# SeoYeonnLee/Video-Chapter-Generation

Hardware: AMD Instinct MI355X
Metric: clip-windows/sec (16f×224²+128tok) train-step at 1/2/4/8 MI355X; % HBM roofline (higher is better)
Workload: dtype bf16; 1 GPU; TwoStream train step: TSM-ResNet-50 + BERT-base + ChapterHead(mlp), B=64 windows/GPU of 16x224^2 frames + 128 tokens, fused clip+AdamW; global_batch=64, seq_len=128, frames=16, resolution=224, text_fill=n_valid ~ U[L/2, L], parallelism=dp1

## Files before the change

include/vcg_hip.h:

```cpp
#ifndef VCG_HIP_H
#define VCG_HIP_H
#include <hip/hip_runtime.h>
#include <stdint.h>
#ifdef __cplusplus
extern "C" {
#endif

#define VCG_API
enum { VCG_F32 = 0, VCG_BF16 = 1 };
enum { VCG_GRAD_F32 = 0x10 };
enum { VCG_OK = 0, VCG_ERR_INVALID = -1, VCG_ERR_UNSUPPORTED = -2, VCG_ERR_HIP = -3 };
enum { VCG_ACT_NONE = 0, VCG_ACT_RELU = 1, VCG_ACT_GELU = 2, VCG_ACT_TANH = 3, VCG_ACT_GELU_BWD = 4 };
enum { VCG_ACT_FLAG_ROUND_PRE = 0x100 };
enum { VCG_ACT_FLAG_WIDE = 0x200 };
enum { VCG_ACT_FLAG_F32_OUT = 0x400 };
VCG_API int vcg_gemm_census_enable(int on);
VCG_API int vcg_gemm_census_size(void);
VCG_API int vcg_gemm_census_get(int i, char* key, int n, long long* count);

VCG_API const char* vcg_last_error(void);
VCG_API int vcg_version(void);
VCG_API int vcg_init(int device);
VCG_API int vcg_finalize(void);
VCG_API int vcg_sync(hipStream_t stream);
VCG_API int vcg_timing_enable(int on);
VCG_API int vcg_timing_query(int kernel_id, double* ms_total, long long* launches, double* flops);
VCG_API int vcg_timing_roofline(int kernel_id, double peak_tflops, double peak_gbs, double* ms_total, double* ideal_ms, double* bytes, double* flops);
VCG_API int vcg_patch_stamps(unsigned long long* out, int n);
VCG_API int vcg_fast_stamps(unsigned long long* out, int n);
VCG_API int vcg_g256_stamps(unsigned long long* out, int n);
VCG_API int vcg_wide_stamps(unsigned long long* out, int n);

VCG_API int vcg_conv_stats_tiles(int M);
VCG_API int vcg_conv_fwd(int dtype, const void* x, const void* w, void* y, float* stats, int N, int H, int W, int C, int Cout, int KH, int KW, int stride, int pad, int tsm_T, int tsm_fold, hipStream_t stream);
VCG_API int vcg_conv_fwd_bias_act(int dtype, const void* x, const void* w, const float* bias, int act, void* y, int N, int H, int W, int C, int Cout, int KH, int KW, int stride, int pad, int tsm_T, int tsm_fold, hipStream_t stream);
VCG_API int vcg_conv_dgrad(int dtype, const void* dy, const void* wt, void* dx, int N, int H, int W, int C, int Cout, int KH, int KW, int stride, int pad, hipStream_t stream);
VCG_API long long vcg_conv_dgrad_bwd_ws_bytes(int C, int Cout, int KH, int KW);
VCG_API long long vcg_conv_dgrad_bwd_p_ws_bytes(int C, int a2_c);
VCG_API int vcg_conv_dgrad_bwd(int dtype, const void* dy, const void* wt, void* g, int N, int H, int W, int C, int Cout, int KH, int KW, int stride, int pad, int tsm_T, int tsm_fold, const void* res, int res_stride, const unsigned char* bits, const void* y, const float* mean, const float* invstd, const float* mscale, const float* mshift, const void* y2, const float* mean2, const float* invstd2, float* ws, long long ws_bytes, float* sum_g, float* sum_gx, float* dgamma, float* dbeta, float* sum_gx2, float* dgamma2, float* dbeta2, const void* a2, int a2_c, float* pg, float* pws, long long pws_bytes, hipStream_t s);
VCG_API long long vcg_conv_wgrad_ws_bytes(int dtype, int N, int H, int W, int C, int Cout, int KH, int KW, int stride, int pad);
VCG_API int vcg_conv_wgrad(int dtype, const void* x, const void* dy, float* dw, int accumulate, float* ws, long long ws_bytes, int N, int H, int W, int C, int Cin, int Cout, int KH, int KW, int stride, int pad, int tsm_T, int tsm_fold, hipStream_t stream);
VCG_API int vcg_conv1x1_bn_res_relu(const void* x, const void* wfold, const float* bias, const void* res, const float* res_scale, const float* res_shift, void* out, unsigned char* bits, int M, int N, int K, hipStream_t stream);
VCG_API int vcg_bn_bwd_fold_weights(const void* wt, int N, int K, const float* mean, const float* invstd, const float* gamma, const float* sum_g, const float* sum_gx, float inv_count, void* wfold, float* bias, hipStream_t stream);
VCG_API long long vcg_bn_apply_colsum_ws_bytes(long long P, int C);
VCG_API int vcg_bn_apply_colsum(const void* y, const float* scale, const float* shift, int relu, void* out, float* colsum, float* ws, long long ws_bytes, long long P, int C, hipStream_t s);
VCG_API long long vcg_bn_apply_gram_ws_bytes(long long P, int C);
VCG_API int vcg_bn_apply_gram(const void* y, const float* scale, const float* shift, const float* mean, const float* invstd, void* out, float* colsum, float* gram, double* g64, float* ws, long long ws_bytes, long long P, int C, hipStream_t s);
VCG_API int vcg_bn_stats_from_gram(const double* g64, const void* w, long long M, int N, int C, float* stats, int mtiles, hipStream_t s);
VCG_API int vcg_bn_finalize_from_gram(const double* g64, const void* w, long long M, int N, int C, const float* gamma,
                                      const float* beta, float* mean, float* invstd, float* scale, float* shift,
                                      float* running_mean, float* running_var, float momentum, float eps,
                                      const float* w32, void* wfold, hipStream_t s);
VCG_API int vcg_conv1x1_stats(const void* x, const void* w, float* stats, int M, int N, int K, hipStream_t stream);
VCG_API int vcg_bn_bwd_sumgx_from_wgrad(const float* P, const void* w, int K, int C, const float* mean, const float* invstd, const float* sum_g, float* sum_gx, float* dgamma, hipStream_t stream);
VCG_API int vcg_bn_bwd_fold_weights_a2(const void* wt, int C, int K, const float* invstd, const float* gamma, const float* sum_g, const float* sum_gx, float inv_count, const float* colsum_a, void* wfold, float* bias, hipStream_t stream);
VCG_API int vcg_bn_bwd_fold_wgrad_a2(const float* P, const float* G, const float* w3, int K, int C, const float* mean, const float* invstd, const float* gamma, const float* sum_g, const float* sum_gx, float inv_count, const float* colsum_a, float* dw, int accumulate, hipStream_t stream);
VCG_API int vcg_conv_dgrad_bwd_bnfold(const void* g, const void* yg, int Ky, const void* wfold, const float* bias, void* out, int N, int H, int W, int C, int Cout, const void* y, const float* mean, const float* invstd, const float* mscale, const float* mshift, float* ws, long long ws_bytes, float* sum_g, float* sum_gx, float* dgamma, float* dbeta, hipStream_t stream);
VCG_API long long vcg_conv_wgrad_bnfold_ws_bytes(int N, int H, int W, int C, int Cout);
// ... 113 lines not shown
```

video-chapter-generation_amd/csrc/igemm.h:

```cpp
#pragma once
#include "common.h"

namespace vcg {

enum { OP_DENSE_K = 0, OP_IM2COL = 1, OP_DGRAD = 2, OP_DENSE_MN = 3, OP_IM2COL_T = 4 };
enum { EPI_STORE = 0, EPI_STATS = 1, EPI_SPLITK = 2, EPI_BWD = 3, EPI_BWD_AFF = 4, EPI_STORE_AUX = 5,
       EPI_BWD_STREAM = 6 };
enum { ACT_NONE = 0, ACT_RELU = 1, ACT_GELU = 2, ACT_TANH = 3, ACT_GELU_BWD = 4 };
enum { ACT_FLAG_ROUND_PRE = 0x100 };
enum { ACT_FLAG_WIDE = 0x200 };
enum { ACT_FLAG_F32_OUT = 0x400 };

template <typename T> struct Cfg;
template <> struct Cfg<float> { static constexpr int VEC = 4, BK = 16, LDK = 20; };
template <> struct Cfg<bf16_t> { static constexpr int VEC = 8, BK = 32, LDK = 40; };

template <typename T, int COLS> struct LdMN {
  static constexpr int v = sizeof(T) == 2 ? (COLS == 128 ? 144 : 80) : (COLS == 128 ? 132 : 68);
};

constexpr bool is_kcontig(int mode) { return mode == OP_DENSE_K || mode == OP_IM2COL || mode == OP_DGRAD; }

struct OpArgs {
  const void* ptr;
// ... 197 lines not shown
            const float mb = red[2 * BN + lc], d = mb - mean, nt = n1 + n2;
            mean += d * (n2 / nt);
            m2 += red[3 * BN + lc] + d * d * (n1 * n2 / nt);
          }
          reinterpret_cast<float2*>(p.stats)[(long long)col * mtiles + mtile] = make_float2(mean, m2);
        }
    }
    if (blockIdx.x == 0 && threadIdx.x == 0)
      reinterpret_cast<float2*>(p.stats)[(long long)p.N * mtiles + mtile] =
          make_float2((float)min(BM, p.M - m0), 0.f);
#pragma unroll
    for (int j = 0; j < NT; ++j) {
      const int n = nbase + j * 16;
#pragma unroll
      for (int i = 0; i < MT; ++i) {
        const int m = mbase + i * 16;
        if (m >= p.M || n >= p.N) continue;
        float v[4] = {acc[i][j][0], acc[i][j][1], acc[i][j][2], acc[i][j][3]};
        store4<T>(Cout + (long long)m * p.ldc + n, v);
      }
    }
  }
}

int run_fast_gemm(GemmParams& p, int amode, int epi, int z, hipStream_t s);
int fast_grid_rows(int M, int N, int z, int epi);
bool fast_bwd_streams(const GemmParams& p);
int wide_gemm_class(const GemmParams& p);
int wide_gemm_class_f32(const GemmParams& p);
int run_gemm_wide(GemmParams& p, int we, hipStream_t s);
int fast_bwd_slots(const GemmParams& p);
int bn_bwd_finalize_launch(const float* partial, int nb, int C, long long ld, int gx_off, float* sum_g, float* sum_gx,
                           float* dgamma, float* dbeta, int accumulate, hipStream_t s);
int run_fast_wgrad(const GemmParams& p, int splits, hipStream_t s, bool dense_b = false);
int wgrad_patch_rows(int dtype, int H, int W, int C, int Cin, int Cout, int KH, int KW, int stride, int pad,
                     int tsm_fold);
int wgrad_patch_splits(int C, int Cout);
int run_rs1x1_bnres(const void* x, const void* wfold, const float* bias, const void* res, void* out, uint8_t* bits,
                    long long M, int N, int K, hipStream_t s);
int run_wgrad_patch(const void* x, const void* dy, float* ws, int N, int H, int W, int C, int Cout, int R,
                    hipStream_t s);
int wgrad_fast_tile_m(int M);
int wgrad_fast_tile_n(int N);

bool gemm256_ok(const GemmParams& p, int amode, int epi, int z);
int run_gemm256(const GemmParams& p, int amode, int epi, hipStream_t s);

}
```

video-chapter-generation_amd/csrc/igemm.hip:

```cpp
#include <cstdio>

#include "igemm.h"

namespace vcg {

template <typename T, int ROWS, int MODE> struct Loader {
  static constexpr int VEC = Cfg<T>::VEC, BK = Cfg<T>::BK;
  static constexpr int NC = ROWS * 4 / 256;
  static constexpr bool KC = is_kcontig(MODE);
  static constexpr int CPR = ROWS / VEC;

  uint4 reg[NC];
  const T* ptr[NC];
  int ra[NC], rb[NC], rc[NC];
  int sub[NC];
  int lds_off[NC];

  __device__ __forceinline__ void init(const OpArgs& a, int row0, int tid) {
    const T* base = reinterpret_cast<const T*>(a.ptr);
#pragma unroll
    for (int j = 0; j < NC; ++j) {
      const int q = tid + j * 256;
      if constexpr (KC) {
        const int row = q >> 2;
// ... 881 lines not shown
  p.K = K;
  p.k_per_split = kps;
  p.a = dense_op(dy, Cout, Cout);
  p.a.bytes = (long long)K * Cout * (dtype == VCG_BF16 ? 2 : 4);
  OpArgs b{};
  b.ptr = x; b.rows = Nn; b.N = N; b.H = H; b.W = W; b.C = C; b.logC = logC;
  b.bytes = (long long)N * H * W * C * (dtype == VCG_BF16 ? 2 : 4);
  b.GH = OH; b.GW = OW; b.KH = KH; b.KW = KW; b.stride = stride; b.pad = pad;
  b.tsm_T = tsm_T > 0 ? tsm_T : 1; b.tsm_fold = tsm_fold;
  b.fd_ghw = make_fastdiv(OH * OW); b.fd_gw = make_fastdiv(OW); b.fd_T = make_fastdiv(b.tsm_T);
  if (pair) {
    b.W = W / 2; b.C = 8; b.logC = 3; b.KW = KWp; b.sw = 1; b.pw = pwp;
  }
  p.b = b;
  p.ws = ws;
  p.alpha = 1.f;
  const int wpr = wgrad_patch_rows(dtype, H, W, C, Cin, Cout, KH, KW, stride, pad, tsm_fold);
  if (wpr > 0) {
    const int wsp = wgrad_patch_splits(C, Cout);
    VCG_REQUIRE(ws_bytes >= (long long)wsp * M * Nn * 4, "workspace too small");
    if (FILE* f = gemm_log())
      fprintf(f, "a=3 b=4 epi=2 M=%d N=%d K=%d z=%d fast=3 conv=%dx%d/%d C=%d\n", M, Nn, K, wsp, KH, KW, stride, C);
    int rc = run_wgrad_patch(x, dy, ws, N, H, W, C, Cout, wpr, stream);
    if (rc) return rc;
    const long long MN = (long long)M * Nn;
    splitk_reduce(stream, ws, wsp, MN,
                       Nn, dw, accumulate, 1, KH, KW, C, Cin, 1.f, KW, 0, pad);
    VCG_LAUNCH_CHECK();
    return VCG_OK;
  }
  FILE* f = fast ? gemm_log() : nullptr;
  if (f)
    fprintf(f, "a=3 b=4 epi=2 M=%d N=%d K=%d z=%d fast=2 conv=%dx%d/%d C=%d\n", M, Nn, K, splits, KH, KW, stride, C);
  int rc;
  if (fast)
    rc = run_fast_wgrad(p, splits, stream);
  else
    rc = dtype == VCG_BF16 ? run_gemm<bf16_t, OP_DENSE_MN, OP_IM2COL_T>(p, EPI_SPLITK, splits, stream)
                           : run_gemm<float, OP_DENSE_MN, OP_IM2COL_T>(p, EPI_SPLITK, splits, stream);
  if (rc) return rc;
  const long long MN = (long long)M * Nn;
  splitk_reduce(stream, ws, splits,
                     MN, Nn, dw, accumulate, pair ? 2 : 1, KH, KW, C, Cin, 1.f, KWp, pwp, pad);
  VCG_LAUNCH_CHECK();
  return VCG_OK;
}

namespace {
__global__ __launch_bounds__(256) void bn_fold_weights_kernel(const bf16_t* __restrict__ wt, int K,
                                                              const float* __restrict__ mean,
                                                              const float* __restrict__ invstd,
                                                              const float* __restrict__ gamma,
                                                              const float* __restrict__ sum_g,
                                                              const float* __restrict__ sum_gx, float ic,
                                                              bf16_t* __restrict__ wf, float* __restrict__ bias) {
  __shared__ float red[256];
  const int n = blockIdx.x, t = threadIdx.x;
  float acc = 0.f;
  for (int k = t; k < K; k += 256) {
    const float is = invstd[k], A = (gamma ? gamma[k] : 1.f) * is;
    const float B = -A * is * sum_gx[k] * ic;
    const float w = bf2f(wt[(long long)n * K + k]);
    const bf16_t wy = f2bf(B * w);
    wf[(long long)n * 2 * K + k] = f2bf(A * w);
    wf[(long long)n * 2 * K + K + k] = wy;
    acc += (-A * sum_g[k] * ic) * w - mean[k] * bf2f(wy);
  }
  red[t] = acc;
  __syncthreads();
  for (int o = 128; o > 0; o >>= 1) {
    if (t < o) red[t] += red[t + o];
    __syncthreads();
  }
  if (t == 0) bias[n] = red[0];
}
// ... 264 lines not shown

VCG_API int vcg_conv_wgrad_bnfold(const void* x, const void* g, const void* yg, const float* mean, const float* invstd,
                                  const float* gamma, const float* sum_g, const float* sum_gx, float inv_count,
                                  const float* colsum_x, float* dw, int accumulate, float* ws, long long ws_bytes, int N,
                                  int H, int W, int C, int Cout, hipStream_t stream) {
  VCG_REQUIRE(x && g && yg && mean && invstd && sum_g && sum_gx && colsum_x && dw, "null argument");
  const int logC = ilog2_exact(C);
  VCG_REQUIRE(logC >= 6 && Cout % 128 == 0, "C must be a power of two >= 64, Cout a multiple of 128");
  int M, Nn, K, splits, kps;
  bool fast;
  wgrad_geometry(VCG_BF16, N, H, W, C, 2 * Cout, 1, 1, 1, 0, &M, &Nn, &K, &splits, &kps, &fast);
  if (!fast || wgrad_fast_tile_m(M) != 128 || (long long)K * Cout * 2 >= 0xFFFFFF00LL) return VCG_ERR_UNSUPPORTED;
  VCG_REQUIRE(ws_bytes >= (long long)splits * M * Nn * 4, "workspace too small");
  GemmParams p{};
  p.M = M;
  p.N = Nn;
  p.K = K;
  p.k_per_split = kps;
  p.a = dense_op(g, Cout, Cout);
  p.a.bytes = (long long)K * Cout * 2;
  p.a.ptr2 = yg;
  p.a.split2 = Cout;
  OpArgs b{};
  b.ptr = x; b.rows = Nn; b.N = N; b.H = H; b.W = W; b.C = C; b.logC = logC;
  b.bytes = (long long)N * H * W * C * 2;
  b.GH = H; b.GW = W; b.KH = 1; b.KW = 1; b.stride = 1; b.pad = 0;
  b.tsm_T = 1; b.tsm_fold = 0;
  b.fd_ghw = make_fastdiv(H * W); b.fd_gw = make_fastdiv(W); b.fd_T = make_fastdiv(1);
  p.b = b;
  p.ws = ws;
  p.alpha = 1.f;
  if (FILE* f = gemm_log())
    fprintf(f, "a=3 b=4 epi=2 M=%d N=%d K=%d z=%d fast=2 conv=1x1/1 C=%d bnfold=1\n", M, Nn, K, splits, C);
  int rc = run_fast_wgrad(p, splits, stream);
  if (rc) return rc;
  const long long MN = (long long)Cout * Nn;
  if ((MN + 255) / 256 < 1024 && splits >= 16)
    hipLaunchKernelGGL(splitk_reduce_bnfold_kernel<8>, dim3((unsigned)((MN * 8 + 255) / 256)), dim3(256), 0, stream,
                       ws, splits, Cout, Nn, mean, invstd, gamma, sum_g, sum_gx, inv_count, colsum_x, dw, accumulate);
  else
    hipLaunchKernelGGL(splitk_reduce_bnfold_kernel<1>, dim3((unsigned)((MN + 255) / 256)), dim3(256), 0, stream, ws,
                       splits, Cout, Nn, mean, invstd, gamma, sum_g, sum_gx, inv_count, colsum_x, dw, accumulate);
  VCG_LAUNCH_CHECK();
  return VCG_OK;
}

VCG_API int vcg_conv1x1_stats(const void* x, const void* w, float* stats, int M, int N, int K, hipStream_t stream) {
  VCG_REQUIRE(x && w && stats, "null argument");
  VCG_REQUIRE(M > 0 && N % 64 == 0 && K % 64 == 0, "N and K must be multiples of 64");
  if (!fast_gemm_enabled() || (long long)M * K * 2 >= 0xFFFFFF00LL) return VCG_ERR_UNSUPPORTED;
  GemmParams p{};
  p.M = M;
  p.N = N;
  p.K = K;
  p.k_per_split = K + 64;
  p.a = dense_op(x, K, M, K, 2);
  p.b = dense_op(w, K, N, K, 2);
  p.C = nullptr;
  p.ldc = N;
  p.alpha = 1.f;
  p.stats = stats;
  if (FILE* f = gemm_log()) {
    fprintf(f, "a=0 b=0 epi=1 M=%d N=%d K=%d z=1 fast=1 conv=1x1/1 C=%d nostore=1\n", M, N, K, K);
    fflush(f);
  }
  const int rc = run_fast_gemm(p, OP_DENSE_K, EPI_STATS, 1, stream);
  return rc < 0 ? VCG_ERR_UNSUPPORTED : rc;
}
// ... 92 lines not shown
  const int splits = choose_splits(M, N, K, dtype == VCG_BF16 ? 32 : 16, VCG_SPLITK_TARGET_DENSE);
  return (long long)splits * M * N * 4;
}

VCG_API int vcg_gemm_splitk(int dtype, int transA, int transB, int M, int N, int K, const void* A, long long lda,
                            const void* B, long long ldb, float* out, int accumulate, float* ws, long long ws_bytes,
                            hipStream_t stream) {
  const int BK = dtype == VCG_BF16 ? 32 : 16;
  int splits = choose_splits(M, N, K, BK, VCG_SPLITK_TARGET_DENSE);
  VCG_REQUIRE(ws_bytes >= (long long)splits * M * N * 4, "workspace too small");
  int kps = (K + splits - 1) / splits;
  kps = (kps + BK - 1) / BK * BK;
  splits = (K + kps - 1) / kps;
  GemmParams p{};
  p.M = M; p.N = N; p.K = K; p.k_per_split = kps;
  p.a = dense_op(A, lda, M);
  p.b = dense_op(B, ldb, N);
  p.ws = ws;
  p.alpha = 1.f;
  int rc;
  const long long a_ext = ((long long)(K - 1) * lda + M) * 2, b_ext = ((long long)(K - 1) * ldb + N) * 2;
  if (dtype == VCG_BF16 && transA && transB && fast_gemm_enabled() &&
      M % 8 == 0 && N % 8 == 0 && lda % 8 == 0 && ldb % 8 == 0 && a_ext < 0xFFFFFF00LL && b_ext < 0xFFFFFF00LL) {
    p.a.bytes = a_ext;
    p.b.bytes = b_ext;
    int fk = (K + splits - 1) / splits;
    fk = (fk + 63) / 64 * 64;
    const int fsplits = (K + fk - 1) / fk;
    p.k_per_split = fk;
    if (FILE* f = gemm_log()) {
      fprintf(f, "a=3 b=3 epi=2 M=%d N=%d K=%d z=%d fast=2 conv=0x0/0 C=0\n", M, N, K, fsplits);
      fflush(f);
    }
    rc = run_fast_wgrad(p, fsplits, stream, true);
    if (rc) return rc;
    const long long MN = (long long)M * N;
    splitk_reduce(stream, ws, fsplits,
                       MN, N, out, accumulate, 0, 1, 1, 1, 1, 1.f, 0, 0, 0);
    VCG_LAUNCH_CHECK();
    return VCG_OK;
  }
#define VCG_SK_CASE(TT)                                                                             \
  if (!transA && !transB) rc = run_gemm<TT, OP_DENSE_K, OP_DENSE_K>(p, EPI_SPLITK, splits, stream);       \
  else if (!transA && transB) rc = run_gemm<TT, OP_DENSE_K, OP_DENSE_MN>(p, EPI_SPLITK, splits, stream);  \
  else if (transA && !transB) rc = run_gemm<TT, OP_DENSE_MN, OP_DENSE_K>(p, EPI_SPLITK, splits, stream);  \
  else rc = run_gemm<TT, OP_DENSE_MN, OP_DENSE_MN>(p, EPI_SPLITK, splits, stream);
  if (dtype == VCG_BF16) { VCG_SK_CASE(bf16_t) } else { VCG_SK_CASE(float) }
#undef VCG_SK_CASE
  if (rc) return rc;
  const long long MN = (long long)M * N;
  splitk_reduce(stream, ws, splits,
                     MN, N, out, accumulate, 0, 1, 1, 1, 1, 1.f, 0, 0, 0);
  VCG_LAUNCH_CHECK();
  return VCG_OK;
}

VCG_API int vcg_gemm_batched(int dtype, int transA, int transB, int M, int N, int K, const void* A, long long lda,
                             long long a_so, long long a_si, const void* B, long long ldb, long long b_so,
                             long long b_si, void* C, long long ldc, long long c_so, long long c_si, int batch_outer,
                             int batch_inner, const float* bias, int act, float alpha, hipStream_t stream) {
  const int VEC = dtype == VCG_BF16 ? 8 : 4;
  VCG_REQUIRE(N % VEC == 0 && ldc % VEC == 0, "N and ldc must be multiples of 16 bytes");
  VCG_REQUIRE(batch_outer > 0 && batch_inner > 0 && M > 0 && N > 0 && K > 0, "empty batched GEMM");
  GemmParams p{};
  p.M = M; p.N = N; p.K = K; p.k_per_split = K + 64;
  const int esz = dtype == VCG_BF16 ? 2 : 4;
  p.a = transA ? dense_op(A, lda, K, M, esz) : dense_op(A, lda, M, K, esz);
  p.b = transB ? dense_op(B, ldb, K, N, esz) : dense_op(B, ldb, N, K, esz);
  p.a.rows = M;
  p.b.rows = N;
// ... 16 lines not shown
```

video-chapter-generation_amd/csrc/igemm_wgrad.hip:

```cpp
#include "igemm.h"

namespace vcg {

namespace {

typedef __attribute__((address_space(3))) void lds_void_t;
typedef __attribute__((address_space(3))) s16x4 lds_s16x4;

constexpr int WBK = 64;

template <int COLS> __device__ __forceinline__ int wswz(int row, int c) {
  if constexpr (COLS == 128) return c ^ (2 * (row & 7));
  else return c ^ (2 * ((row >> 1) & 3));
}

template <int COLS, bool GATHER> struct MNLoader {
  static constexpr int CPR = COLS / 8;
  static constexpr int RPI = 64 / CPR;
  static constexpr int NI = WBK / RPI / 4;
  __amdgpu_buffer_rsrc_t rsrc;
  uint32_t oob;
  int row[NI];
  int col[NI];
  int kh[NI], kw[NI], dt[NI];
// ... 82 lines not shown
      const uint32_t voff = ok ? (uint32_t)e * 2u : oob;
      bf16_t* slice = lds + (wave * NI + q) * 512;
      __builtin_amdgcn_raw_ptr_buffer_load_lds(rsrc, (lds_void_t*)slice, 16, voff, 0, 0, 0);
      okm |= ok ? (1u << q) : 0u;
    }
    return okm;
  }
};

typedef __attribute__((address_space(3))) char lds_char;
__device__ __forceinline__ uint32_t lds_addr(const bf16_t* p) { return (uint32_t)(uintptr_t)(const lds_char*)p; }

template <int COLS> __device__ __forceinline__ void wfrag_issue(s16x4& lo, s16x4& hi, const bf16_t* lds, int r0,
                                                                int lane, int s2) {
  const int g = lane >> 4, i = lane & 15;
  const int q = i >> 2, pp = i & 3;
  const int cl = r0 + 4 * pp;
  const int k0 = 32 * s2 + 4 * g + q, k1 = k0 + 16;
  const uint32_t a0 = lds_addr(lds + k0 * COLS + 8 * wswz<COLS>(k0, cl >> 3) + (cl & 7));
  const uint32_t a1 = lds_addr(lds + k1 * COLS + 8 * wswz<COLS>(k1, cl >> 3) + (cl & 7));
  asm volatile("ds_read_b64_tr_b16 %0, %1" : "=v"(lo) : "v"(a0) : "memory");
  asm volatile("ds_read_b64_tr_b16 %0, %1" : "=v"(hi) : "v"(a1) : "memory");
}
__device__ __forceinline__ s16x8 cat8(const s16x4& lo, const s16x4& hi) {
  return s16x8{lo[0], lo[1], lo[2], lo[3], hi[0], hi[1], hi[2], hi[3]};
}
__device__ __forceinline__ void lgkm0() {
  asm volatile("s_waitcnt lgkmcnt(0)" ::: "memory");
  __builtin_amdgcn_sched_barrier(0);
}

__device__ __forceinline__ constexpr int wvm(int n) { return (n & 0xF) | (0x7 << 4) | (0xF << 8) | (((n >> 4) & 3) << 14); }

template <int BM, int BN, bool BG>
__global__ __launch_bounds__(256) __attribute__((amdgpu_waves_per_eu(2))) void wgrad_fast_kernel(GemmParams p) {
  constexpr int MT = BM / 32, NT = BN / 32;
  constexpr int AE = WBK * BM, BE = WBK * BN;
  constexpr int NLD = MNLoader<BM, false>::NI + MNLoader<BN, BG>::NI;
  __shared__ __attribute__((aligned(1024))) bf16_t smem[2 * (AE + BE)];
  bf16_t* As = smem;
  bf16_t* Bs = smem + 2 * AE;

  const int tid = threadIdx.x, lane = tid & 63, wave = __builtin_amdgcn_readfirstlane(tid >> 6);
  const int wm = wave >> 1, wn = wave & 1;
  const int nx = (p.N + BN - 1) / BN, mtiles = (p.M + BM - 1) / BM, per = nx * mtiles;
  const int sidx = blockIdx.x >> 3;
  const int split = (sidx / per) * 8 + (blockIdx.x & 7);
  if (split >= p.batch_inner) return;
  const int t = sidx % per;
  const int bx = t % nx, bym = t / nx;
  const int n0 = bx * BN, m0 = bym * BM;
  const int kb = split * p.k_per_split;
  const int ke = min(p.K, kb + p.k_per_split);
  const int ntiles = (ke - kb + WBK - 1) / WBK;

  MNLoader<BM, false> la;
  MNLoader<BN, BG> lb;
  la.init(p.a, m0, p.M, kb, wave, lane);
  lb.init(p.b, n0, p.N, kb, wave, lane);

  f32x4 acc[MT][NT];
#pragma unroll
  for (int i = 0; i < MT; ++i)
#pragma unroll
    for (int j = 0; j < NT; ++j) acc[i][j] = f32x4{0.f, 0.f, 0.f, 0.f};

  if (ntiles > 0) {
    la.issue(p.a, kb, ke, As, wave);
    lb.issue(p.b, kb, ke, Bs, wave);
  }
  for (int t = 0; t < ntiles; ++t) {
    const int cur = t & 1;
    if (t + 1 < ntiles) {
      la.issue(p.a, kb + (t + 1) * WBK, ke, As + (cur ^ 1) * AE, wave);
      lb.issue(p.b, kb + (t + 1) * WBK, ke, Bs + (cur ^ 1) * BE, wave);
      __builtin_amdgcn_s_waitcnt(wvm(NLD));
    } else {
      __builtin_amdgcn_s_waitcnt(wvm(0));
    }
    __builtin_amdgcn_s_barrier();
    const bf16_t* Ac = As + cur * AE;
    const bf16_t* Bc = Bs + cur * BE;
    s16x4 al[2][MT], ah[2][MT], bl[2][NT], bh[2][NT];
#pragma unroll
    for (int s2 = 0; s2 < 2; ++s2) {
#pragma unroll
      for (int i = 0; i < MT; ++i) wfrag_issue<BM>(al[s2][i], ah[s2][i], Ac, wm * (BM / 2) + i * 16, lane, s2);
#pragma unroll
      for (int j = 0; j < NT; ++j) wfrag_issue<BN>(bl[s2][j], bh[s2][j], Bc, wn * (BN / 2) + j * 16, lane, s2);
      if (s2 == 0) lgkm0();
    }
#pragma unroll
    for (int s2 = 0; s2 < 2; ++s2) {
      if (s2 == 1) lgkm0();
#pragma unroll
      for (int i = 0; i < MT; ++i)
#pragma unroll
        for (int j = 0; j < NT; ++j)
          acc[i][j] = __builtin_amdgcn_mfma_f32_16x16x32_bf16(cat8(bl[s2][j], bh[s2][j]), cat8(al[s2][i], ah[s2][i]),
                                                              acc[i][j], 0, 0, 0);
    }
    __builtin_amdgcn_s_waitcnt(0xC07F);
    __builtin_amdgcn_s_barrier();
  }

  const int g = lane >> 4, ci = lane & 15;
  const int mbase = m0 + wm * (BM / 2) + ci, nbase = n0 + wn * (BN / 2) + 4 * g;
  float* ws = p.ws + (long long)split * p.M * p.N;
#pragma unroll
  for (int i = 0; i < MT; ++i) {
    const int m = mbase + i * 16;
    if (m >= p.M) continue;
#pragma unroll
    for (int j = 0; j < NT; ++j) {
      const int n = nbase + j * 16;
      if (n < p.N) *reinterpret_cast<f32x4*>(ws + (long long)m * p.N + n) = acc[i][j];
    }
  }
}

template <int BM, int BN, bool BG> int launch_wgrad(const GemmParams& p0, int splits, hipStream_t s) {
  GemmParams p = p0;
  p.batch_inner = splits;
  const long long per = (long long)((p.N + BN - 1) / BN) * ((p.M + BM - 1) / BM);
  const long long wgs = (splits + 7) / 8 * 8 * per;
  VCG_REQUIRE(wgs < (1LL << 31), "wgrad grid too large");
  const int tk = timing_begin(s);
  hipLaunchKernelGGL((wgrad_fast_kernel<BM, BN, BG>), dim3((unsigned)wgs), dim3(256), 0, s, p);
  if (census_on()) { char t_[96]; snprintf(t_, sizeof(t_), "wgrad_fast %dx%d bg%d z%d", BM, BN, (int)BG, splits); census_add(t_, p.M, p.N, p.K); }
  timing_end(tk, s, TIMING_WGRAD, 2.0 * p.M * p.N * (double)p.K,
             (double)p.a.bytes + (double)p.b.bytes + 4.0 * p.M * (double)p.N);
  VCG_LAUNCH_CHECK();
  return VCG_OK;
}

constexpr int WP_SL = 32;
constexpr int WP_RING = 3;
constexpr int WP_GRID = 256;

struct WPatchGeom {
  int H, W, R, TM, PW, NP, NS, tiles, TPI;
  int C, CO, nct, nch, nsplit;
};

__device__ __forceinline__ int wp_swz(int row, int c) { return c ^ (2 * ((row >> 1) & 3)); }

template <int OFF> __device__ __forceinline__ void tr_read_at(s16x4& v, uint32_t addr) {
  asm volatile("ds_read_b64_tr_b16 %0, %1 offset:%2" : "=v"(v) : "v"(addr), "i"(OFF) : "memory");
}

template <int PW, int KS>
__global__ __launch_bounds__(256) __attribute__((amdgpu_waves_per_eu(1, 1)))
void wgrad3x3_patch_kernel(const bf16_t* __restrict__ x, const bf16_t* __restrict__ dy, float* __restrict__ ws,
                           uint32_t xbytes, uint32_t dybytes, WPatchGeom g) {
  constexpr int PE = WP_SL * 512, YE = 32 * KS * 64;
  constexpr int NIP = 8 + KS;
  __shared__ __attribute__((aligned(1024))) bf16_t smem[WP_RING * (PE + YE)];
  bf16_t* Ps = smem;
  bf16_t* Ys = smem + WP_RING * PE;
  const int tid = threadIdx.x, lane = tid & 63, wave = __builtin_amdgcn_readfirstlane(tid >> 6);
  const int lg = lane >> 4, li = lane & 15, q = li >> 2, pp = li & 3;
  const int b = blockIdx.x, rest = b >> 3;
  const int chb = rest % g.nch, split = (rest / g.nch) * 8 + (b & 7);
  const int ci_t = chb % g.nct, co_t = chb / g.nct;
  const int t0 = (int)(((long long)g.tiles * split) / g.nsplit);
// ... 91 lines not shown
#pragma unroll
    for (int st = 0; st < KS; ++st) {
      const int b2 = st & 1;
      asm volatile("s_waitcnt lgkmcnt(0)" ::: "memory");
      __builtin_amdgcn_sched_barrier(0);
      if (st + 1 < KS) reads(st + 1, b2 ^ 1);
#pragma unroll
      for (int t = 0; t < 9; ++t) {
        const s16x8 bf = cat8(bl[b2][t], bh[b2][t]);
#pragma unroll
        for (int ct = 0; ct < 4; ++ct)
          acc[ct][t] = __builtin_amdgcn_mfma_f32_16x16x32_bf16(cat8(al[b2][ct], ah[b2][ct]), bf, acc[ct][t], 0, 0, 0);
      }
      __builtin_amdgcn_sched_barrier(0);
    }
    asm volatile("s_waitcnt lgkmcnt(0)" ::: "memory");
  }
  const int NC = 9 * g.C;
  float* slab = ws + (long long)split * g.CO * NC;
#pragma unroll
  for (int ct = 0; ct < 4; ++ct)
#pragma unroll
    for (int t = 0; t < 9; ++t)
#pragma unroll
      for (int r = 0; r < 4; ++r)
        slab[(long long)(64 * co_t + 16 * ct + 4 * lg + r) * NC + t * g.C + 64 * ci_t + 16 * wave + li] = acc[ct][t][r];
}

}

int wgrad_fast_tile_m(int M) { return M >= 128 ? 128 : 64; }
int wgrad_fast_tile_n(int N) { return N > 64 ? 128 : 64; }

int run_fast_wgrad(const GemmParams& p, int splits, hipStream_t s, bool dense_b) {
  const int bm = wgrad_fast_tile_m(p.M), bn = wgrad_fast_tile_n(p.N);
  if (dense_b) {
    if (bm == 128 && bn == 128) return launch_wgrad<128, 128, false>(p, splits, s);
    if (bm == 128) return launch_wgrad<128, 64, false>(p, splits, s);
    if (bn == 128) return launch_wgrad<64, 128, false>(p, splits, s);
    return launch_wgrad<64, 64, false>(p, splits, s);
  }
  if (bm == 128 && bn == 128) return launch_wgrad<128, 128, true>(p, splits, s);
  if (bm == 128) return launch_wgrad<128, 64, true>(p, splits, s);
  if (bn == 128) return launch_wgrad<64, 128, true>(p, splits, s);
  return launch_wgrad<64, 64, true>(p, splits, s);
}

int wgrad_patch_rows(int dtype, int H, int W, int C, int Cin, int Cout, int KH, int KW, int stride, int pad,
                     int tsm_fold) {
  static int en = -1;
  if (en < 0) {
    const char* e = getenv("VCG_WGRAD_PATCH");
    en = (e && e[0] == '0') ? 0 : (e && e[0] == '1') ? 1 : 2;
  }
  if (!en || dtype != VCG_BF16 || C != Cin || C % 64 != 0 || Cout % 64 != 0 || C > 512 || Cout > 512 || KH != 3 ||
      KW != 3 || stride != 1 || pad != 1 || tsm_fold != 0)
    return 0;
  if (en == 1 && (C != 64 || Cout != 64)) return 0;
  if (W + 2 > 64 || W < 14) return 0;
  const int pw = W + 2 <= 16 ? 16 : W + 2 <= 32 ? 32 : 64;
  for (int R = 128 / W; R >= 1; --R)
    if ((R + 2) * pw <= 8 * WP_SL && H % R == 0) return R;
  return 0;
}

static int wp_grid(int C, int Cout) {
  const int nch = (C / 64) * (Cout / 64);
  int nsplit = WP_GRID / nch;
  nsplit = nsplit < 8 ? 8 : nsplit & ~7;
  return nsplit * nch;
}

int wgrad_patch_splits(int C, int Cout) { return wp_grid(C, Cout) / ((C / 64) * (Cout / 64)); }

template <int PW>
static void launch_wgrad_patch(const void* x, const void* dy, float* ws, uint32_t xb, uint32_t yb, const WPatchGeom& g,
                               int grid, hipStream_t s) {
  if (census_on()) { char t_[96]; snprintf(t_, sizeof(t_), "wgrad3x3_patch pw%d tm%d", PW, g.TM); census_add(t_, 0, 0, 0); }
  if (g.TM <= 64)
    hipLaunchKernelGGL((wgrad3x3_patch_kernel<PW, 2>), dim3(grid), dim3(256), 0, s, (const bf16_t*)x,
                       (const bf16_t*)dy, ws, xb, yb, g);
  else
    hipLaunchKernelGGL((wgrad3x3_patch_kernel<PW, 4>), dim3(grid), dim3(256), 0, s, (const bf16_t*)x,
                       (const bf16_t*)dy, ws, xb, yb, g);
}

int run_wgrad_patch(const void* x, const void* dy, float* ws, int N, int H, int W, int C, int Cout, int R,
                    hipStream_t s) {
  WPatchGeom g;
  const int pw = W + 2 <= 16 ? 16 : W + 2 <= 32 ? 32 : 64;
  g.H = H; g.W = W; g.R = R; g.TM = R * W; g.PW = pw; g.NP = (R + 2) * pw; g.NS = (g.NP + 7) / 8;
  g.TPI = H / R; g.tiles = N * g.TPI;
  g.C = C; g.CO = Cout; g.nct = C / 64; g.nch = (C / 64) * (Cout / 64);
  const int grid = wp_grid(C, Cout);
  g.nsplit = grid / g.nch;
  const long long xb = (long long)N * H * W * C * 2, yb = (long long)N * H * W * Cout * 2;
  VCG_REQUIRE(xb < 0xFFFFFF00LL && yb < 0xFFFFFF00LL, "wgrad patch: x / dy must be below 4 GB");
  VCG_REQUIRE(g.TM <= 128, "wgrad patch: tile rows");
  const int tk = timing_begin(s);
  if (pw == 64) launch_wgrad_patch<64>(x, dy, ws, (uint32_t)xb, (uint32_t)yb, g, grid, s);
  else if (pw == 32) launch_wgrad_patch<32>(x, dy, ws, (uint32_t)xb, (uint32_t)yb, g, grid, s);
  else launch_wgrad_patch<16>(x, dy, ws, (uint32_t)xb, (uint32_t)yb, g, grid, s);
  timing_end(tk, s, TIMING_WGRAD, 2.0 * Cout * 9 * C * (double)N * H * W, (double)xb + (double)yb + 4.0 * Cout * 9 * C);
  VCG_LAUNCH_CHECK();
  return VCG_OK;
}

}
```

video-chapter-generation_amd/vcg_hip/ops.py:

```python
import os

import torch

from . import _lib

F32, BF16 = 0, 1
ACT_NONE, ACT_RELU, ACT_GELU, ACT_TANH, ACT_GELU_BWD = 0, 1, 2, 3, 4
ACT_FLAG_ROUND_PRE = 0x100
ACT_FLAG_WIDE = 0x200
ACT_FLAG_F32_OUT = 0x400
GRAD_F32 = 0x10

_DT = {torch.float32: F32, torch.bfloat16: BF16}


def dt_code(dtype):
    try:
        return _DT[dtype]
    except KeyError:
        raise TypeError(f"unsupported storage dtype {dtype}; expected float32 or bfloat16")


def torch_dtype(precision):
    return {"fp32": torch.float32, "bf16": torch.bfloat16}[precision]
# ... 14 lines not shown
def _chk(t, dtype=None, name="tensor"):
    if not t.is_cuda:
        raise RuntimeError(f"{name} must be on the GPU (libvcg_hip has no CPU path)")
    if not t.is_contiguous():
        raise RuntimeError(f"{name} must be contiguous")
    if dtype is not None and t.dtype != dtype:
        raise RuntimeError(f"{name} has dtype {t.dtype}, expected {dtype}")


def ws(nbytes, device):
    return torch.empty((max(int(nbytes), 4) + 3) // 4, dtype=torch.float32, device=device)


def conv_out_hw(H, W, KH, KW, stride, pad):
    return (H + 2 * pad - KH) // stride + 1, (W + 2 * pad - KW) // stride + 1


TIMING_FAST_GEMM, TIMING_WGRAD, TIMING_GENERIC_GEMM, TIMING_PATCH_CONV, TIMING_WIDE_GEMM = 0, 1, 2, 3, 4


def gemm_census_enable(on):
    _lib.call("vcg_gemm_census_enable", int(bool(on)))


def gemm_census():
    import ctypes
    out = {}
    for i in range(_lib.query("vcg_gemm_census_size")):
        buf = ctypes.create_string_buffer(256)
        n = ctypes.c_longlong()
        _lib.call("vcg_gemm_census_get", i, buf, 256, ctypes.addressof(n))
        out[buf.value.decode()] = n.value
    return out


def timing_enable(on):
    _lib.call("vcg_timing_enable", int(bool(on)))


def timing_query(kernel_id):
    import ctypes
    ms, n, fl = ctypes.c_double(), ctypes.c_longlong(), ctypes.c_double()
    _lib.call("vcg_timing_query", int(kernel_id), ctypes.addressof(ms), ctypes.addressof(n), ctypes.addressof(fl))
    return ms.value, n.value, fl.value


def timing_roofline(kernel_id, peak_tflops, peak_gbs):
    import ctypes
    ms, ideal, nb, fl = ctypes.c_double(), ctypes.c_double(), ctypes.c_double(), ctypes.c_double()
    _lib.call("vcg_timing_roofline", int(kernel_id), float(peak_tflops), float(peak_gbs), ctypes.addressof(ms),
              ctypes.addressof(ideal), ctypes.addressof(nb), ctypes.addressof(fl))
    return ms.value, ideal.value, nb.value, fl.value


def stats_tiles(M):
    return _lib.query("vcg_conv_stats_tiles", M)


def stats_buffer(Cout, M, device):
    return torch.empty((Cout + 1, stats_tiles(M), 2), dtype=torch.float32, device=device)


def conv_fwd(x, w, N, H, W, C, Cout, KH, KW, stride, pad, tsm_T=0, tsm_fold=0, stats=None, out=None):
    _chk(x, name="x")
    if stats is not None:
        OH_, OW_ = conv_out_hw(H, W, KH, KW, stride, pad)
# ... 747 lines not shown
```

Baseline: 921.7 clip-windows/sec.

## Split wgrad workgroups into two K groups reducing partials through LDS

```diff
diff --git a/include/vcg_hip.h b/include/vcg_hip.h
--- a/include/vcg_hip.h
+++ b/include/vcg_hip.h
@@ -24,6 +24,7 @@
 VCG_API int vcg_finalize(void);
 VCG_API int vcg_sync(hipStream_t stream);
 VCG_API int vcg_timing_enable(int on);
+VCG_API int vcg_wgrad_kgroups(int mode);
 VCG_API int vcg_timing_query(int kernel_id, double* ms_total, long long* launches, double* flops);
 VCG_API int vcg_timing_roofline(int kernel_id, double peak_tflops, double peak_gbs, double* ms_total, double* ideal_ms, double* bytes, double* flops);
 VCG_API int vcg_patch_stamps(unsigned long long* out, int n);
diff --git a/video-chapter-generation_amd/csrc/igemm.h b/video-chapter-generation_amd/csrc/igemm.h
--- a/video-chapter-generation_amd/csrc/igemm.h
+++ b/video-chapter-generation_amd/csrc/igemm.h
@@ -253,7 +253,7 @@
 int fast_bwd_slots(const GemmParams& p);
 int bn_bwd_finalize_launch(const float* partial, int nb, int C, long long ld, int gx_off, float* sum_g, float* sum_gx,
                            float* dgamma, float* dbeta, int accumulate, hipStream_t s);
-int run_fast_wgrad(const GemmParams& p, int splits, hipStream_t s, bool dense_b = false);
+int run_fast_wgrad(const GemmParams& p, int splits, hipStream_t s, int* slabs, bool dense_b = false);
 int wgrad_patch_rows(int dtype, int H, int W, int C, int Cin, int Cout, int KH, int KW, int stride, int pad,
                      int tsm_fold);
 int wgrad_patch_splits(int C, int Cout);
diff --git a/video-chapter-generation_amd/csrc/igemm.hip b/video-chapter-generation_amd/csrc/igemm.hip
--- a/video-chapter-generation_amd/csrc/igemm.hip
+++ b/video-chapter-generation_amd/csrc/igemm.hip
@@ -937,15 +937,15 @@
   FILE* f = fast ? gemm_log() : nullptr;
   if (f)
     fprintf(f, "a=3 b=4 epi=2 M=%d N=%d K=%d z=%d fast=2 conv=%dx%d/%d C=%d\n", M, Nn, K, splits, KH, KW, stride, C);
-  int rc;
+  int rc, slabs = splits;
   if (fast)
-    rc = run_fast_wgrad(p, splits, stream);
+    rc = run_fast_wgrad(p, splits, stream, &slabs);
   else
     rc = dtype == VCG_BF16 ? run_gemm<bf16_t, OP_DENSE_MN, OP_IM2COL_T>(p, EPI_SPLITK, splits, stream)
                            : run_gemm<float, OP_DENSE_MN, OP_IM2COL_T>(p, EPI_SPLITK, splits, stream);
   if (rc) return rc;
   const long long MN = (long long)M * Nn;
-  splitk_reduce(stream, ws, splits,
+  splitk_reduce(stream, ws, slabs,
                      MN, Nn, dw, accumulate, pair ? 2 : 1, KH, KW, C, Cin, 1.f, KWp, pwp, pad);
   VCG_LAUNCH_CHECK();
   return VCG_OK;
@@ -1276,8 +1276,10 @@
   p.alpha = 1.f;
   if (FILE* f = gemm_log())
     fprintf(f, "a=3 b=4 epi=2 M=%d N=%d K=%d z=%d fast=2 conv=1x1/1 C=%d bnfold=1\n", M, Nn, K, splits, C);
-  int rc = run_fast_wgrad(p, splits, stream);
+  int slabs = splits;
+  int rc = run_fast_wgrad(p, splits, stream, &slabs);
   if (rc) return rc;
+  splits = slabs;
   const long long MN = (long long)Cout * Nn;
   if ((MN + 255) / 256 < 1024 && splits >= 16)
     hipLaunchKernelGGL(splitk_reduce_bnfold_kernel<8>, dim3((unsigned)((MN * 8 + 255) / 256)), dim3(256), 0, stream,
@@ -1436,10 +1438,11 @@
       fprintf(f, "a=3 b=3 epi=2 M=%d N=%d K=%d z=%d fast=2 conv=0x0/0 C=0\n", M, N, K, fsplits);
       fflush(f);
     }
-    rc = run_fast_wgrad(p, fsplits, stream, true);
+    int slabs = fsplits;
+    rc = run_fast_wgrad(p, fsplits, stream, &slabs, true);
     if (rc) return rc;
     const long long MN = (long long)M * N;
-    splitk_reduce(stream, ws, fsplits,
+    splitk_reduce(stream, ws, slabs,
                        MN, N, out, accumulate, 0, 1, 1, 1, 1, 1.f, 0, 0, 0);
     VCG_LAUNCH_CHECK();
     return VCG_OK;
diff --git a/video-chapter-generation_amd/csrc/igemm_wgrad.hip b/video-chapter-generation_amd/csrc/igemm_wgrad.hip
--- a/video-chapter-generation_amd/csrc/igemm_wgrad.hip
+++ b/video-chapter-generation_amd/csrc/igemm_wgrad.hip
@@ -138,27 +138,49 @@
 
 __device__ __forceinline__ constexpr int wvm(int n) { return (n & 0xF) | (0x7 << 4) | (0xF << 8) | (((n >> 4) & 3) << 14); }
 
-template <int BM, int BN, bool BG>
-__global__ __launch_bounds__(256) __attribute__((amdgpu_waves_per_eu(2))) void wgrad_fast_kernel(GemmParams p) {
+template <int BM, int BN, bool BG, int KG, bool STAG>
+__global__ __launch_bounds__(256 * KG) __attribute__((amdgpu_waves_per_eu(2))) void wgrad_fast_kernel(GemmParams p) {
+  static_assert(KG == 1 || KG == 2, "one or two K groups");
+  static_assert(KG == 2 || !STAG, "staggering needs two groups");
   constexpr int MT = BM / 32, NT = BN / 32;
   constexpr int AE = WBK * BM, BE = WBK * BN;
+  constexpr int GE = 2 * (AE + BE);
   constexpr int NLD = MNLoader<BM, false>::NI + MNLoader<BN, BG>::NI;
-  __shared__ __attribute__((aligned(1024))) bf16_t smem[2 * (AE + BE)];
-  bf16_t* As = smem;
-  bf16_t* Bs = smem + 2 * AE;
-
-  const int tid = threadIdx.x, lane = tid & 63, wave = __builtin_amdgcn_readfirstlane(tid >> 6);
+  static_assert(BM * BN * 4 <= GE * 2, "group 1 parks its accumulators in its stages");
+  __shared__ __attribute__((aligned(1024))) bf16_t smem[KG * GE];
+
+  const int tid = threadIdx.x, lane = tid & 63, wv = __builtin_amdgcn_readfirstlane(tid >> 6);
+  const int grp = KG == 2 ? wv >> 2 : 0, wave = wv & 3;
+  bf16_t* As = smem + grp * GE;
+  bf16_t* Bs = As + 2 * AE;
   const int wm = wave >> 1, wn = wave & 1;
   const int nx = (p.N + BN - 1) / BN, mtiles = (p.M + BM - 1) / BM, per = nx * mtiles;
   const int sidx = blockIdx.x >> 3;
-  const int split = (sidx / per) * 8 + (blockIdx.x & 7);
-  if (split >= p.batch_inner) return;
-  const int t = sidx % per;
+  const int nsplit = p.batch_inner;
+  const int nslab = (nsplit + KG - 1) / KG;
+  int slab, t;
+  if (KG == 2 && nslab <= 4) {
+    const int lq = nslab <= 1 ? 0 : nslab <= 2 ? 1 : 2, x = blockIdx.x & 7;
+    slab = x & ((1 << lq) - 1);
+    t = (sidx << (3 - lq)) + (x >> lq);
+    if (slab >= nslab || t >= per) return;
+  } else {
+    slab = (sidx / per) * 8 + (blockIdx.x & 7);
+    if (slab >= nslab) return;
+    t = sidx % per;
+  }
   const int bx = t % nx, bym = t / nx;
   const int n0 = bx * BN, m0 = bym * BM;
+  const int split = KG * slab + grp;
   const int kb = split * p.k_per_split;
   const int ke = min(p.K, kb + p.k_per_split);
-  const int ntiles = (ke - kb + WBK - 1) / WBK;
+  const int ntiles = split < nsplit ? (ke - kb + WBK - 1) / WBK : 0;
+  int nloop = ntiles;
+  if constexpr (KG == 2) {
+    const int kb0 = KG * slab * p.k_per_split;
+    nloop = (min(p.K, kb0 + p.k_per_split) - kb0 + WBK - 1) / WBK;
+    nloop = max(nloop, ntiles);
+  }
 
   MNLoader<BM, false> la;
   MNLoader<BN, BG> lb;
@@ -175,7 +197,10 @@
     la.issue(p.a, kb, ke, As, wave);
     lb.issue(p.b, kb, ke, Bs, wave);
   }
-  for (int t = 0; t < ntiles; ++t) {
+  if constexpr (STAG) {
+    if (grp == 1) __builtin_amdgcn_s_barrier();
+  }
+  for (int t = 0; t < nloop; ++t) {
     const int cur = t & 1;
     if (t + 1 < ntiles) {
       la.issue(p.a, kb + (t + 1) * WBK, ke, As + (cur ^ 1) * AE, wave);
@@ -187,32 +212,80 @@
     __builtin_amdgcn_s_barrier();
     const bf16_t* Ac = As + cur * AE;
     const bf16_t* Bc = Bs + cur * BE;
-    s16x4 al[2][MT], ah[2][MT], bl[2][NT], bh[2][NT];
-#pragma unroll
-    for (int s2 = 0; s2 < 2; ++s2) {
-#pragma unroll
-      for (int i = 0; i < MT; ++i) wfrag_issue<BM>(al[s2][i], ah[s2][i], Ac, wm * (BM / 2) + i * 16, lane, s2);
-#pragma unroll
-      for (int j = 0; j < NT; ++j) wfrag_issue<BN>(bl[s2][j], bh[s2][j], Bc, wn * (BN / 2) + j * 16, lane, s2);
-      if (s2 == 0) lgkm0();
-    }
-#pragma unroll
-    for (int s2 = 0; s2 < 2; ++s2) {
-      if (s2 == 1) lgkm0();
+    if constexpr (!STAG) {
+      if (KG == 1 || t < ntiles) {
+        s16x4 al[2][MT], ah[2][MT], bl[2][NT], bh[2][NT];
+#pragma unroll
+        for (int s2 = 0; s2 < 2; ++s2) {
+#pragma unroll
+          for (int i = 0; i < MT; ++i) wfrag_issue<BM>(al[s2][i], ah[s2][i], Ac, wm * (BM / 2) + i * 16, lane, s2);
+#pragma unroll
+          for (int j = 0; j < NT; ++j) wfrag_issue<BN>(bl[s2][j], bh[s2][j], Bc, wn * (BN / 2) + j * 16, lane, s2);
+          if (s2 == 0) lgkm0();
+        }
+#pragma unroll
+        for (int s2 = 0; s2 < 2; ++s2) {
+          if (s2 == 1) lgkm0();
+#pragma unroll
+          for (int i = 0; i < MT; ++i)
+#pragma unroll
+            for (int j = 0; j < NT; ++j)
+              acc[i][j] = __builtin_amdgcn_mfma_f32_16x16x32_bf16(cat8(bl[s2][j], bh[s2][j]),
+                                                                  cat8(al[s2][i], ah[s2][i]), acc[i][j], 0, 0, 0);
+        }
+      }
+      __builtin_amdgcn_s_waitcnt(0xC07F);
+      __builtin_amdgcn_s_barrier();
+    } else {
+      if (t < ntiles) {
+        s16x4 al[2][MT], ah[2][MT], bl[2][NT], bh[2][NT];
+#pragma unroll
+        for (int s2 = 0; s2 < 2; ++s2) {
+#pragma unroll
+          for (int i = 0; i < MT; ++i) wfrag_issue<BM>(al[s2][i], ah[s2][i], Ac, wm * (BM / 2) + i * 16, lane, s2);
+#pragma unroll
+          for (int j = 0; j < NT; ++j) wfrag_issue<BN>(bl[s2][j], bh[s2][j], Bc, wn * (BN / 2) + j * 16, lane, s2);
+        }
+        lgkm0();
+        __builtin_amdgcn_s_barrier();
+#pragma unroll
+        for (int s2 = 0; s2 < 2; ++s2)
+#pragma unroll
+          for (int i = 0; i < MT; ++i)
+#pragma unroll
+            for (int j = 0; j < NT; ++j)
+              acc[i][j] = __builtin_amdgcn_mfma_f32_16x16x32_bf16(cat8(bl[s2][j], bh[s2][j]),
+                                                                  cat8(al[s2][i], ah[s2][i]), acc[i][j], 0, 0, 0);
+      } else {
+        __builtin_amdgcn_s_barrier();
+      }
+    }
+  }
+  if constexpr (STAG) {
+    if (grp == 0) __builtin_amdgcn_s_barrier();
+  }
+
+  if constexpr (KG == 2) {
+    f32x4* park = reinterpret_cast<f32x4*>(smem + GE) + (tid & 255);
+    if (grp == 1) {
 #pragma unroll
       for (int i = 0; i < MT; ++i)
 #pragma unroll
-        for (int j = 0; j < NT; ++j)
-          acc[i][j] = __builtin_amdgcn_mfma_f32_16x16x32_bf16(cat8(bl[s2][j], bh[s2][j]), cat8(al[s2][i], ah[s2][i]),
-                                                              acc[i][j], 0, 0, 0);
-    }
-    __builtin_amdgcn_s_waitcnt(0xC07F);
+        for (int j = 0; j < NT; ++j) park[(i * NT + j) * 256] = acc[i][j];
+    }
+    asm volatile("s_waitcnt lgkmcnt(0)" ::: "memory");
     __builtin_amdgcn_s_barrier();
+    asm volatile("" ::: "memory");
+    if (grp == 1) return;
+#pragma unroll
+    for (int i = 0; i < MT; ++i)
+#pragma unroll
+      for (int j = 0; j < NT; ++j) acc[i][j] = acc[i][j] + park[(i * NT + j) * 256];
   }
 
   const int g = lane >> 4, ci = lane & 15;
   const int mbase = m0 + wm * (BM / 2) + ci, nbase = n0 + wn * (BN / 2) + 4 * g;
-  float* ws = p.ws + (long long)split * p.M * p.N;
+  float* ws = p.ws + (long long)slab * p.M * p.N;
 #pragma unroll
   for (int i = 0; i < MT; ++i) {
     const int m = mbase + i * 16;
@@ -225,18 +298,40 @@
   }
 }
 
-template <int BM, int BN, bool BG> int launch_wgrad(const GemmParams& p0, int splits, hipStream_t s) {
+int g_kgroups = -1;
+
+template <int BM, int BN, bool BG> constexpr int kgroups_default() {
+  if (BG && BM == 128 && BN == 64) return 2;
+  if (BG && BM == 64 && BN == 128) return 1;
+  if (BG && BM == 64 && BN == 64) return 2;
+  if (!BG && BM == 128 && BN == 128) return 2;
+  return 0;
+}
+
+template <int BM, int BN, bool BG> int launch_wgrad(const GemmParams& p0, int splits, hipStream_t s, int* slabs) {
   GemmParams p = p0;
   p.batch_inner = splits;
+  const int mode = g_kgroups < 0 ? kgroups_default<BM, BN, BG>() : g_kgroups;
+  const int kg = mode ? 2 : 1, nslab = (splits + kg - 1) / kg;
   const long long per = (long long)((p.N + BN - 1) / BN) * ((p.M + BM - 1) / BM);
-  const long long wgs = (splits + 7) / 8 * 8 * per;
+  long long wgs = (nslab + 7) / 8 * 8 * per;
+  if (kg == 2 && nslab <= 4) {
+    const int r = nslab <= 1 ? 8 : nslab <= 2 ? 4 : 2;
+    wgs = (per + r - 1) / r * 8;
+  }
   VCG_REQUIRE(wgs < (1LL << 31), "wgrad grid too large");
   const int tk = timing_begin(s);
-  hipLaunchKernelGGL((wgrad_fast_kernel<BM, BN, BG>), dim3((unsigned)wgs), dim3(256), 0, s, p);
+  if (mode == 0)
+    hipLaunchKernelGGL((wgrad_fast_kernel<BM, BN, BG, 1, false>), dim3((unsigned)wgs), dim3(256), 0, s, p);
+  else if (mode == 1)
+    hipLaunchKernelGGL((wgrad_fast_kernel<BM, BN, BG, 2, false>), dim3((unsigned)wgs), dim3(512), 0, s, p);
+  else
+    hipLaunchKernelGGL((wgrad_fast_kernel<BM, BN, BG, 2, true>), dim3((unsigned)wgs), dim3(512), 0, s, p);
   if (census_on()) { char t_[96]; snprintf(t_, sizeof(t_), "wgrad_fast %dx%d bg%d z%d", BM, BN, (int)BG, splits); census_add(t_, p.M, p.N, p.K); }
   timing_end(tk, s, TIMING_WGRAD, 2.0 * p.M * p.N * (double)p.K,
              (double)p.a.bytes + (double)p.b.bytes + 4.0 * p.M * (double)p.N);
   VCG_LAUNCH_CHECK();
+  *slabs = nslab;
   return VCG_OK;
 }
 
@@ -394,18 +489,18 @@
 int wgrad_fast_tile_m(int M) { return M >= 128 ? 128 : 64; }
 int wgrad_fast_tile_n(int N) { return N > 64 ? 128 : 64; }
 
-int run_fast_wgrad(const GemmParams& p, int splits, hipStream_t s, bool dense_b) {
+int run_fast_wgrad(const GemmParams& p, int splits, hipStream_t s, int* slabs, bool dense_b) {
   const int bm = wgrad_fast_tile_m(p.M), bn = wgrad_fast_tile_n(p.N);
   if (dense_b) {
-    if (bm == 128 && bn == 128) return launch_wgrad<128, 128, false>(p, splits, s);
-    if (bm == 128) return launch_wgrad<128, 64, false>(p, splits, s);
-    if (bn == 128) return launch_wgrad<64, 128, false>(p, splits, s);
-    return launch_wgrad<64, 64, false>(p, splits, s);
-  }
-  if (bm == 128 && bn == 128) return launch_wgrad<128, 128, true>(p, splits, s);
-  if (bm == 128) return launch_wgrad<128, 64, true>(p, splits, s);
-  if (bn == 128) return launch_wgrad<64, 128, true>(p, splits, s);
-  return launch_wgrad<64, 64, true>(p, splits, s);
+    if (bm == 128 && bn == 128) return launch_wgrad<128, 128, false>(p, splits, s, slabs);
+    if (bm == 128) return launch_wgrad<128, 64, false>(p, splits, s, slabs);
+    if (bn == 128) return launch_wgrad<64, 128, false>(p, splits, s, slabs);
+    return launch_wgrad<64, 64, false>(p, splits, s, slabs);
+  }
+  if (bm == 128 && bn == 128) return launch_wgrad<128, 128, true>(p, splits, s, slabs);
+  if (bm == 128) return launch_wgrad<128, 64, true>(p, splits, s, slabs);
+  if (bn == 128) return launch_wgrad<64, 128, true>(p, splits, s, slabs);
+  return launch_wgrad<64, 64, true>(p, splits, s, slabs);
 }
 
 int wgrad_patch_rows(int dtype, int H, int W, int C, int Cin, int Cout, int KH, int KW, int stride, int pad,
@@ -469,3 +564,9 @@
 }
 
 }
+
+VCG_API int vcg_wgrad_kgroups(int mode) {
+  const int prev = vcg::g_kgroups;
+  vcg::g_kgroups = mode < 0 ? -1 : mode > 2 ? 2 : mode;
+  return prev;
+}
diff --git a/video-chapter-generation_amd/vcg_hip/ops.py b/video-chapter-generation_amd/vcg_hip/ops.py
--- a/video-chapter-generation_amd/vcg_hip/ops.py
+++ b/video-chapter-generation_amd/vcg_hip/ops.py
@@ -70,6 +70,10 @@
         _lib.call("vcg_gemm_census_get", i, buf, 256, ctypes.addressof(n))
         out[buf.value.decode()] = n.value
     return out
+
+
+def wgrad_kgroups(mode):
+    return _lib.query("vcg_wgrad_kgroups", int(mode))
 
 
 def timing_enable(on):
```

Result: no change. 921.1 clip-windows/sec (-0.1%).
